# ssmit1986/BayesianInference

Measured on AMD Instinct MI355X. Metric: GP log-marg-lik evals/sec at N=32768, d=8; Cholesky TFLOP/s vs fp64 peak, higher is better.
Workload: dtype f64

## Files before the change

### bayesianinference_amd/csrc/gp_kernels.h

```cpp
#pragma once
#include <hip/hip_runtime.h>
#include <stdint.h>

#include <type_traits>

namespace gphip {

#define GP_RTC_ABI 7
#ifdef GP_D
#define GP_DIM(x) (GP_D)
#else
#define GP_DIM(x) (x)
#endif
constexpr int TB = 128;
constexpr long TS = (long)TB * TB;

__host__ __device__ __forceinline__ long tile_index(int ti, int tj, int R) {
    return (long)tj * R - ((long)tj * (tj - 1)) / 2 + (ti - tj);
}
__host__ __device__ __forceinline__ int panel_slot(int tj, int nt, int panel) {
    return tj >= nt ? (nt + panel - 1) / panel : tj / panel;
}
constexpr int SLOTP = 16;

// ... 708 lines not shown
        return sf2 * __builtin_amdgcn_exp2f(-fmaxf(u, 0.f));
    } else if (KT == 2) {
        const float q = fmaxf(u, 1e-30f);
        const float s3 = q * __builtin_amdgcn_rsqf(q);
        return sf2 * (1.0f + s3) * __builtin_amdgcn_exp2f(s3 * -1.4426950408889634f);
    } else if (KT == 3) {
        const float q = fmaxf(u, 0.f) * inv_alpha;
        return sf2 * __builtin_amdgcn_exp2f(-alpha * __builtin_amdgcn_logf(1.0f + q));
    } else {
        const float q = fmaxf(u, 1e-30f);
        const float s5 = q * __builtin_amdgcn_rsqf(q);
        return sf2 * (1.0f + s5 + q * (1.0f / 3.0f)) * __builtin_amdgcn_exp2f(s5 * -1.4426950408889634f);
    }
}

template <typename T, int KS, int KT>
__global__ __launch_bounds__(256, 2) void kbuild_mfma_kernel(KBuildMArgs<T> m) {
    const KBuildArgs<T>& a = m.b;
    constexpr int NQ = 16 / (int)sizeof(T);
    constexpr int IBR = 16 * NQ;
    constexpr int NIB = TB / IBR;
    typedef T vec_t __attribute__((ext_vector_type(NQ)));
    typedef typename Num<T>::acc_t acc_t;
    typedef typename Num<T>::pair_t pair_t;
    extern __shared__ double lds_raw[];
    const int tid = threadIdx.x, lane = tid & 63, wave = tid >> 6;
    const int slot = blockIdx.y;
    int ti, tj;
    if (a.mode == 0) {
        tri_decode(blockIdx.x + a.t0, a.nt_i, ti, tj);
    } else {
        ti = blockIdx.x % a.nt_i;
        tj = blockIdx.x / a.nt_i;
    }
    if (a.own_world > 0) {
        const int owner = (tj == a.nt_j) ? 0 : (tj / a.own_panel) % a.own_world;
        if (owner != a.own_rank) return;
    }
    const double* sp = a.slotp + (long)slot * SLOTP;
    if (sp[SP_MFMA] == 0.0) return;
    const T sf2 = (T)sp[0], sn2 = (T)sp[1], mu = (T)sp[2];
    const T alpha = (T)sp[SP_ALPHA1], inv_sf2 = (T)(1.0 / sp[0]), inv_alpha = (T)(1.0 / sp[SP_ALPHA1]);
    const T coff = (T)sp[SP_OFFSET];
    const long ldo = (a.mode == 0) ? (long)TB : a.ld;
    T* out = a.out + (long)slot * a.bstride +
             ((a.mode == 0) ? (tile_index(ti, tj, a.nt_i) + (a.adj ? a.adj[panel_slot(tj, a.nt_j, a.own_panel)] : 0l)) * TS
                            : (long)tj * TB * a.ld + (long)ti * TB);
    if (a.mode == 0 && ti == a.nt_i - 1) {
        const int r0 = 2 * lane;
        for (int jj = wave * 32; jj < wave * 32 + 32; ++jj) {
            const int gj = tj * TB + jj;
            pair_t v;
            v.x = (T)0;
            v.y = (T)0;
            if (lane == 0 && tj < a.nt_j && gj < a.n_j)
                v.x = a.y[gj] - (a.pw_mean ? a.pw_mean[(long)slot * a.pw_bstride + gj] : mu);
            *reinterpret_cast<pair_t*>(out + (long)jj * ldo + r0) = v;
        }
        return;
    }
    const int d = a.d;
    const int ks = KS > 0 ? KS : (d + 3) / 4, kr = 4 * ks;
    constexpr int KSR = KS > 0 ? KS : KB_LDS_MAXD / 4;
    constexpr bool JREG = sizeof(T) == 8;
    T* xjs = reinterpret_cast<T*>(lds_raw);
    T* xis = xjs + (JREG ? 0 : kr * KM_LDP);
    T* nrm = xis + kr * KM_LDP;
    const double* etab = reinterpret_cast<const double*>(nrm + 2 * TB);
    if (sizeof(T) == 8) {
        double* et = const_cast<double*>(etab);
        for (int idx = tid; idx < EXP_TAB; idx += 256) et[idx] = sp[0] * a.exp2tab[idx];
    }
    const double* ie = m.inv_ell + (long)slot * d;
    const double cs = KmScale<T, KT>::v;
    {
        const int side = tid >> 7, p = tid & 127;
        const T* src = side ? m.xri + (long)ti * TB + p : m.xrj + (long)tj * TB + p;
        const long np = side ? a.npad_i : a.npad_j;
        T* dst = (side ? xis : xjs) + p;
        double n2 = 0.0;
        for (int dd = 0; dd < d; ++dd) {
            const T v = (T)(((double)src[(long)dd * np] - m.centre[dd]) * (ie[dd] * cs));
            n2 = __builtin_fma((double)v, (double)v, n2);
            if (side) dst[dd * KM_LDP] = v;
            else if (!JREG) dst[dd * KM_LDP] = (T)-2 * v;
        }
        if (side || !JREG)
            for (int dd = d; dd < kr; ++dd) dst[dd * KM_LDP] = (T)0;
        nrm[side * TB + p] = (T)n2;
    }
    const int c = lane & 15, g = lane >> 4;
    T avr[2][JREG ? KSR : 1];
    if constexpr (JREG) {
#pragma unroll
        for (int jbi = 0; jbi < 2; ++jbi)
#pragma unroll
            for (int s = 0; s < KSR; ++s) {
                const int k = 4 * s + g;
                T v = (T)0;
                if (k < d)
                    v = (T)-2 * (T)(((double)m.xrj[(long)k * a.npad_j + (long)tj * TB + (wave + 4 * jbi) * 16 + c] - m.centre[k]) * (ie[k] * cs));
                avr[jbi][s] = v;
            }
    }
    __syncthreads();

    const bool edge = (a.mode == 0) ? (ti == tj || (ti + 1) * TB > a.n_i)
                                    : ((ti + 1) * TB > a.n_i || (tj + 1) * TB > a.n_j);
#pragma unroll
    for (int jbi = 0; jbi < 2; ++jbi)
#pragma unroll 1
    for (int ib = 0; ib < NIB; ++ib) {
        const int jb = wave + 4 * jbi;
        const int j0 = jb * 16, i0 = ib * IBR + NQ * c;
        const vec_t nai = *reinterpret_cast<const vec_t*>(nrm + TB + i0);
        acc_t acc[NQ];
#pragma unroll
        for (int r = 0; r < 4; ++r) {
            const T nbj = nrm[j0 + Num<T>::drow(g, r)];
#pragma unroll
            for (int q = 0; q < NQ; ++q) acc[q][r] = nai[q] + nbj;
        }
#pragma unroll
        for (int s = 0; s < KSR; ++s) {
            if (KS > 0 || s < ks) {
                const T av = JREG ? avr[jbi][JREG ? s : 0] : xjs[(4 * s + g) * KM_LDP + j0 + c];
                const vec_t bv = *reinterpret_cast<const vec_t*>(xis + (4 * s + g) * KM_LDP + i0);
#pragma unroll
                for (int q = 0; q < NQ; ++q) acc[q] = Num<T>::mfma(av, bv[q], acc[q]);
            }
        }
        const int gi0 = ti * TB + i0;
#pragma unroll
        for (int r = 0; r < 4; ++r) {
            const int jc = j0 + Num<T>::drow(g, r);
            vec_t v;
#pragma unroll
            for (int q = 0; q < NQ; ++q) v[q] = km_value<KT>(acc[q][r], sf2, etab, alpha, inv_sf2, inv_alpha) + coff;
            if (edge) {
                const int gj = tj * TB + jc;
#pragma unroll
                for (int q = 0; q < NQ; ++q) {
                    const int gi = gi0 + q;
                    if (a.mode == 0) {
                        if (gi == gj) v[q] += a.pw_nug ? a.pw_nug[(long)slot * a.pw_bstride + gj] : sn2;
                        if (gj >= a.n_j || gi >= a.n_i) v[q] = (gi == gj) ? (T)1 : (T)0;
                    } else if (gj >= a.n_j || gi >= a.n_i) {
                        v[q] = (T)0;
                    }
                }
            }
            *reinterpret_cast<vec_t*>(out + (long)jc * ldo + i0) = v;
        }
    }
}

#ifdef GPHIP_TIMING
__device__ long long* g_stamp_buf;
#define GP_STAMP(i) do { if (threadIdx.x == 0 && g_stamp_buf) g_stamp_buf[(long)blockIdx.x * 64 + (i)] = wall_clock64(); } while (0)
#else
#define GP_STAMP(i) do { } while (0)
#endif

__device__ __forceinline__ double fast_rsqrt(double x) {
    const double y = __builtin_amdgcn_rsq(x);
    const double hy = 0.5 * y;
// ... 475 lines not shown
    const long* c_adj; int c_adj_panel;
    int K;
    int r0, r1, c0, c1;
    int tri;
    int nrect;
    int ntiles;
    int swizzle;
    int super;
    int mode;
    int ktri;
    int grp_stride, grp_width, grp_count;
    int thin_row;
    int fuse_b;
    T* fuse_W; double* fuse_partial; int* fuse_info; const double* fuse_slotp; int fuse_nt;
    int skip_upper;
};

__device__ __forceinline__ void blocked_tri_decode(int p, int H, int& u, int& v) {
    const int Sf = H >> 3;
    auto prefix = [&](int J) { return (long)J * (8 * H - 28) - 32l * J * (J - 1); };
    const double b = 8.0 * H + 4.0;
    const double disc = b * b - 128.0 * (double)p;
    int J = (int)((b - __builtin_sqrt(disc > 0.0 ? disc : 0.0)) * (1.0 / 64.0));
    if (J < 0) J = 0;
    if (J > Sf) J = Sf;
    while (J > 0 && prefix(J) > p) --J;
    while (J < Sf && prefix(J + 1) <= p) ++J;
    const int q = p - (int)prefix(J);
    if (J == Sf) {
        int uu, vv;
// ... 10 lines not shown
        return;
    }
    const int below = H - 8 * J - 8, nfull = below >> 3, q2 = q - 36;
    int grp = q2 >> 6;
    if (grp < nfull) {
        const int w = q2 & 63;
        u = 8 * J + 8 + 8 * grp + (w & 7);
        v = 8 * J + (w >> 3);
    } else {
        const int rl = below & 7, w = q2 - 64 * nfull;
        u = 8 * J + 8 + 8 * nfull + w % rl;
        v = 8 * J + w / rl;
    }
}

template <typename T>
__device__ __forceinline__ void gemm_tile_decode(const GemmArgs<T>& g, int t, int r0, int c0, int nrect, int& ti, int& tj) {
    const int H = g.r1 - r0;
    if (!g.tri || t < nrect) {
        tj = c0 + t / H;
        ti = r0 + t % H;
    } else {
        int u, v;
        tri_decode(t - nrect, H, u, v);
        ti = r0 + u;
        tj = r0 + v;
    }
}

template <typename T> __device__ __forceinline__ int lds_off(int k, int row);
template <> __device__ __forceinline__ int lds_off<double>(int k, int row) { return k * LDT + row; }
template <> __device__ __forceinline__ int lds_off<float>(int k, int row) {
    return ((k >> 2) * 2 + (k & 1)) * LDP + ((k >> 1) & 1) * TB + row;
}

#ifndef GP_DIAG
#define GP_DIAG 0
#endif
template <typename T, int ROLE, int NWI, int NWJ, int NBUF>
__global__ __launch_bounds__(64 * NWI * NWJ, (NWI * NWJ == 4) ? 2 : 4) void gemm_nt_kernel(GemmArgs<T> g) {
    constexpr int NW = NWI * NWJ, FI = 8 / NWI, FJ = 8 / NWJ;
    const bool c_tiled = g.c_R > 0, a_tiled = g.a_R > 0, b_tiled = g.b_R > 0;
    extern __shared__ double smem_raw[];
    T* smem = reinterpret_cast<T*>(smem_raw);
    typedef typename Num<T>::acc_t acc_t;
    constexpr int GK = Num<T>::GK;
    constexpr int STAGE = STAGE_BYTES / (int)sizeof(T);
    constexpr int JOFF = STAGE / 2;
    constexpr bool F64 = sizeof(T) == 8;
    const int tid = threadIdx.x, lane = tid & 63, wave = tid >> 6;
    const int wi = wave % NWI, wj = wave / NWI;
    int slot = blockIdx.y;
    int bid = blockIdx.x;
    int ti, tj;
    int r0 = g.r0, c0 = g.c0, nrect = g.nrect, ntiles = g.ntiles;
// ... 16 lines not shown
        nrect = 0;
        ntiles = ntc * H - ntc * (ntc - 1) / 2;
        if (bid >= ntiles) return;
    }
    if (g.super == 2) {
        const int H = g.r1 - g.r0;
        {
            const int nx = 8, n = ntiles;
            const int q = n / nx, rem = n % nx, x = bid % nx, o = bid / nx;
            bid = (x < rem ? x * (q + 1) : rem * (q + 1) + (x - rem) * q) + o;
        }
        int u, v;
        blocked_tri_decode(bid, H, u, v);
        ti = g.r0 + u;
        tj = g.r0 + v;
    } else {
        if (g.swizzle) {
            const int nx = 8, n = ntiles;
            const int q = n / nx, rem = n % nx, x = bid % nx, o = bid / nx;
            bid = (x < rem ? x * (q + 1) : rem * (q + 1) + (x - rem) * q) + o;
        }
        gemm_tile_decode(g, bid, r0, c0, nrect, ti, tj);
    }
    ti = __builtin_amdgcn_readfirstlane(ti);
    tj = __builtin_amdgcn_readfirstlane(tj);
    slot = __builtin_amdgcn_readfirstlane(slot);

    const long koff = g.ktri ? (long)ti * TB : 0;
    const T* Abase = g.A + (long)slot * g.a_bstride;
    const T* Bbase = g.B + (long)slot * g.b_bstride;
// ... 61 lines not shown
        }
    };

    const long ldc = c_tiled ? (long)TB : g.ldc;
    T* Cg = g.C + (long)slot * g.c_bstride +
            (c_tiled ? (tile_index(ti, tj, g.c_R) + (g.c_adj ? g.c_adj[panel_slot(tj, g.c_R - 1, g.c_adj_panel)] : 0l)) * TS
                     : (long)tj * TB * g.ldc + (long)ti * TB) +
            (long)(wj * (16 * FJ)) * ldc + wi * (16 * FI) + (lane & 15);
    const int l4 = lane >> 4;
    const int nk = (g.K - (int)koff) / GK;
    const bool from_zero = (ROLE == 2) || (ROLE == 3 && g.mode == 1);
    acc_t acc[FJ][FI];
    int ny = FI;
    if (NW == 4) {
        const int uwi = uw % NWI, uwj = uw / NWI;
        if (g.thin_row == ti) ny = (uwi == 0) ? 1 : 0;
        else if (g.skip_upper && g.tri && ti == tj && uwi == 0 && uwj == 1) ny = 0;
    }
    auto load_c = [&](auto nyc) {
        constexpr int NY = decltype(nyc)::value;
#pragma unroll
        for (int x = 0; x < FJ; ++x)
#pragma unroll
            for (int y = 0; y < FI; ++y) {
                if (from_zero || (GP_DIAG & 2) || y >= NY) {
                    acc[x][y] = (acc_t){0, 0, 0, 0};
                } else {
#pragma unroll
                    for (int r = 0; r < 4; ++r)
                        acc[x][y][r] = Cg[(long)(x * 16 + Num<T>::drow(l4, r)) * ldc + y * 16];
                }
            }
    };
    auto load_frags = [&](int buf, int kk, T* fi, T* fj) {
        const T* Is = smem + buf * STAGE + wi * (16 * FI) + (lane & 15);
        const T* Js = smem + buf * STAGE + JOFF;
        const int k = 4 * kk + l4;
#pragma unroll
        for (int f = 0; f < FI; ++f) fi[f] = Is[lds_off<T>(k, f * 16)];
#pragma unroll
        for (int f = 0; f < FJ; ++f) {
            const int jrow = wj * (16 * FJ) + f * 16 + (lane & 15);
            if (ROLE == 3) {
                constexpr int G = 16 / (int)sizeof(T);
                fj[f] = Js[jrow * GK + G * ((k / G) ^ (jrow & 7)) + (k % G)];
            } else {
                fj[f] = Js[lds_off<T>(k, jrow)];
// ... 35 lines not shown
            load_frags(buf, kk, fi, fj);
            mfma_block(fi, fj, std::integral_constant<int, FI>{}, kb * GK + 4 * kk);
        }
    };
    if constexpr (NBUF == 2) {
        constexpr int NKK = GK / 4;
        static_assert(NKK % 2 == 0, "fragment set parity must repeat every stage");
        auto pipeline = [&](auto nyc) {
            constexpr int NY = decltype(nyc)::value;
            T fa[2][FI], fb[2][FJ];
#ifdef GP_STAGGER
            if (ROLE == 0 && (blockIdx.x & 256) && blockIdx.x < 512)
                for (int i = 0; i < GP_STAGGER; ++i) __builtin_amdgcn_s_sleep(127);
#endif
            stage(0, 0);
            load_c(nyc);
            asm volatile("s_waitcnt vmcnt(0)" ::: "memory");
            __syncthreads();
            if (NY > 0) load_frags(0, 0, fa[0], fb[0]);
            for (int kb = 0; kb < nk; ++kb) {
                const int cur = kb & 1;
                if (kb + 1 < nk && !((GP_DIAG & 1) && kb >= 1)) stage(kb + 1, cur ^ 1);
                if (NY > 0) {
#pragma unroll
                    for (int kk = 0; kk + 1 < NKK; ++kk) {
                        pin_frags(fa[kk & 1], fb[kk & 1]);
                        __builtin_amdgcn_sched_barrier(0);
                        load_frags(cur, kk + 1, fa[(kk + 1) & 1], fb[(kk + 1) & 1]);
                        __builtin_amdgcn_sched_barrier(0);
                        mfma_block(fa[kk & 1], fb[kk & 1], nyc, kb * GK + 4 * kk);
                        __builtin_amdgcn_sched_barrier(0);
// ... 1310 lines not shown
```

### bayesianinference_amd/csrc/gphip.hip

```cpp
#include "gp_kernels.h"
#include "gp_trsv.h"
#include "rccl_dyn.h"
#include "rtc_dyn.h"

#include <hip/hip_ext.h>

#include <algorithm>
#include <chrono>
#include <cctype>
#include <cmath>
#include <cstdio>
#include <cstdlib>
#include <cstring>
#include <mutex>
#include <string>
#include <vector>

#include "../../include/gphip.h"

using namespace gphip;

namespace {

constexpr double LOG_TWO_PI = 1.8378770664093454835606594728112;
// ... 93 lines not shown
    Buf dExp2;
    Buf dCentre;
    std::vector<double> x_centre, x_half;
    int kbuild_mfma = 1, kbuild_mfma_bound = 512, kbuild_mfma_digits = 9;
    double test_ratio = 0.0;
    int slots = 0;
    Buf dA, dXs, dW;
    Buf dDinv;
    Buf dW64;
    unsigned long w64_gen = ~0ul;
    Buf dLT, dW64T;
    unsigned long lt_gen = ~0ul;
    Buf dInvEll, dSlotp, dPartial, dRes, dInfo;
    Buf hInvEll, hSlotp, hRes, hInfo;
    int panel = 4, profile = 0, swizzle = 1, max_slots = 256, lookahead = 1;
    int supertile = 2;
    int latency_gemm = 1;
    static constexpr int latency_tiles = 256;
    int latency_max_nt = 48;
    int dataflow = 1, dataflow_max_nt = 96;
    int dataflow_max_slots = -1;
    int dataflow_max_tasks = 34000;
    int dataflow_fine_nt = 96;
    int panel_left = -1;
    int fuse_option = 1;
    int grad_potri = 1;
    int grad_batch_slots = 0;
    int grad_batch_max_n = 7168;
    int grad_batch_last = 0, grad_batch_route = 0;
    Buf dKinvB;
    int predict_df_max_nt = 256;
// ... 362 lines not shown
bool use_dataflow(const gphip_ctx* h, int nslots);
inline int few_slots(const gphip_ctx* h) { return h->dataflow_max_slots < 0 ? 8 : h->dataflow_max_slots; }
hipEvent_t sync_event(gphip_ctx* h);

void queue_custom_prep(gphip_ctx* h, int nslots) {
    if (!h->custom) return;
    const void* x = h->dXt.p;
    int npad = (int)h->Npad, n = (int)h->N, d = (int)h->d, ncp = std::max(h->ncp, 1);
    const double* cp = h->dCustomP.as<double>();
    double* sp = h->dSlotp.as<double>();
    void* params[] = {&x, &npad, &n, &d, &cp, &ncp, &sp};
    (void)hipModuleLaunchKernel(h->f_cprep, (unsigned)nslots, 1, 1, 256, 1, 1, 0, h->cs, params, nullptr);
}

template <typename T>
int queue_build(gphip_ctx* h, int nslots) {
    const long tot = (long)h->d * h->Npad;
    int gx = (int)((tot + 255) / 256);
    if (gx > 1024) gx = 1024;
    if (h->theta_packed) {
        ThetaPack tp;
        memcpy(tp.v, h->hInvEll.as<double>(), (size_t)nslots * h->d * 8);
        memcpy(tp.v + (size_t)nslots * h->d, h->hSlotp.as<double>(), (size_t)nslots * SLOTP * 8);
        hipLaunchKernelGGL(k_scale_theta<T>, dim3(gx, nslots), dim3(256), 0, h->cs, (const T*)h->dXt.p, (T*)h->dXs.p, tp,
                           h->dInvEll.as<double>(), h->dSlotp.as<double>(), h->dInfo.as<int>(), (int)h->d, (int)h->Npad, nslots);
    } else {
        hipLaunchKernelGGL(k_scale<T>, dim3(gx, nslots), dim3(256), 0, h->cs, (const T*)h->dXt.p, (T*)h->dXs.p,
                           h->dInvEll.as<double>(), (int)h->d, (int)h->Npad);
    }
    if (h->nl2 > 0)
        hipLaunchKernelGGL(k_scale<T>, dim3(gx, nslots), dim3(256), 0, h->cs, (const T*)h->dXt.p, (T*)h->dXs2.p, h->dInvEll2.as<double>(),
                           (int)h->d, (int)h->Npad);
    queue_custom_prep(h, nslots);
    KBuildArgs<T> a{};
    a.ks = h->ks; a.xi2 = a.xj2 = (const T*)h->dXs2.p;
    a.out = (T*)h->dA.p; a.ld = TB; a.bstride = h->slot_elems;
    a.xi = (const T*)h->dXs.p; a.xj = (const T*)h->dXs.p; a.xi_bstride = a.xj_bstride = tot;
    a.npad_i = a.npad_j = (int)h->Npad; a.n_i = a.n_j = (int)h->N;
    a.y = (const T*)h->dY.p; a.slotp = h->dSlotp.as<double>(); a.d = (int)h->d; a.mode = 0; a.exp2tab = h->dExp2.as<double>();
    a.nt_i = (int)h->Nt + 1; a.nt_j = (int)h->Nt;
    a.own_panel = h->panel; a.own_world = h->dist_world; a.own_rank = h->dist_rank;
    if (h->dist_world > 0) { a.out = (T*)h->dist_base; a.adj = h->dDistAdj.as<long>(); }
    a.pw_nug = h->pw_nug_on ? (const T*)h->dPwNug.p : nullptr;
    a.pw_mean = h->pw_mean_on ? (const T*)h->dPwMean.p : nullptr;
    a.pw_bstride = h->Npad;
    const long ntiles = (long)(h->Nt + 1) * (h->Nt + 2) / 2;
    ProfScope ps(h, 0, 0.0, (double)sizeof(T) * nslots * ((double)h->N * (h->N + 1) / 2 + (double)h->N * h->d));
    launch_kbuild<T>(h, a, dim3((unsigned)ntiles, nslots), (const T*)h->dXt.p, (const T*)h->dXt.p);
    return 0;
}

template <typename T>
struct Opnd {
    const T* p; long ld; long bs; int R; int k0;
    const long* adj = nullptr; int adj_panel = 0;
    int lower = 0;
};
template <typename T>
Opnd<T> cm(const T* p, long ld, long bs) { return Opnd<T>{p, ld, bs, 0, 0}; }
template <typename T>
Opnd<T> wb(const T* W, int b, long lrs) {
    Opnd<T> o{W + (long)b * TB * TB - (long)b * TB, TB, lrs, 0, 0};
    o.lower = 1;
    return o;
}
template <typename T>
Opnd<T> tl(const gphip_ctx* h, int k0 = 0, bool all_slots = true) {
    return Opnd<T>{(const T*)(h->ws_override ? h->ws_override : h->dA.p), TB, all_slots ? (long)h->slot_elems : 0l, (int)h->R, k0};
}

template <typename T>
size_t potrf_lds();

template <typename T>
bool launch_gemm(gphip_ctx* h, int cls, Opnd<T> Co, Opnd<T> Ao, Opnd<T> Bo, int K, int r0, int r1, int c0, int c1, int tri,
                 int nslots, int mode = 0, int ktri = 0, int thin_row = -1, int fuse_b = -1, int groups = 1, int grp_stride = 0,
                 int grp_width = 0) {
    GemmArgs<T> g{};
    g.grp_stride = groups > 1 ? grp_stride : 0;
    g.grp_width = grp_width;
    g.grp_count = groups;
    g.mode = mode;
    g.ktri = ktri;
    g.thin_row = h->thin_tiles ? thin_row : -1;
    g.skip_upper = (h->thin_tiles && thin_row >= 0 && tri && mode == 0 && !ktri) ? 1 : 0;
    g.C = const_cast<T*>(Co.p); g.ldc = Co.ld; g.c_bstride = Co.bs; g.c_R = Co.R;
    g.c_adj = Co.adj; g.c_adj_panel = Co.adj_panel;
    g.b_lower = Bo.lower;
    g.A = Ao.p; g.lda = Ao.ld; g.a_bstride = Ao.bs; g.a_R = Ao.R; g.a_k0 = Ao.k0;
    g.B = Bo.p; g.ldb = Bo.ld; g.b_bstride = Bo.bs; g.b_R = Bo.R; g.b_k0 = Bo.k0;
    g.K = K; g.r0 = r0; g.r1 = r1; g.c0 = c0; g.c1 = c1; g.tri = tri;
    const int H = r1 - r0, W = c1 - c0;
    if (H <= 0 || W <= 0) return false;
    if (!tri) {
        g.nrect = H * W;
        g.ntiles = H * W;
    } else {
        int nrc = r0 - c0;
        if (nrc > W) nrc = W;
        const int ntc = W - nrc;
        g.nrect = nrc * H;
        g.ntiles = g.nrect + ntc * H - ntc * (ntc - 1) / 2;
    }
    g.swizzle = h->swizzle && g.ntiles >= 64 && !ktri;
    int grid_x = g.ntiles;
    if (tri && r0 == c0 && W == H && h->supertile >= 2 && H >= 16 && mode == 0 && groups == 1 && (nslots == 1 || h->supertile == 3)) {
        g.super = 2;
    }
    double flops = 2.0 * TB * TB * (double)K * g.ntiles * nslots;
    if (g.grp_stride > 0) {
        double fl = 0.0;
        long tiles = 0;
        for (int q = 0; q < groups; ++q) {
            const int a0 = c0 + q * grp_stride, a1 = std::min(a0 + grp_width, c1);
            const int Hq = r1 - a0, wq = a1 - a0;
            tiles += (long)wq * Hq - (long)wq * (wq - 1) / 2;
            const double a = (double)a0 * TB, b = std::min((double)a1 * TB, (double)h->N);
            const double cnt = b > a ? b - a : 0.0;
            fl += 2.0 * (double)K * (cnt * (double)h->N - (a + b - 1.0) * cnt / 2.0);
        }
        long dense = 0;
        for (int q = 0; q < groups; ++q) {
            const int a0 = c0 + q * grp_stride, wq = std::min(grp_width, c1 - a0), Hq = r1 - a0;
            dense += (long)wq * Hq - (long)wq * (wq - 1) / 2;
        }
        g.nrect = 0;
        g.ntiles = (int)dense;
        flops = cls == 4 ? fl : 2.0 * TB * TB * (double)K * (double)tiles;
    } else if (cls == 4 && tri && r0 == c0) {
        const double a = (double)c0 * TB, b = std::min((double)c1 * TB, (double)h->N);
        const double cnt = b > a ? b - a : 0.0;
        flops = 2.0 * (double)K * (cnt * (double)h->N - (a + b - 1.0) * cnt / 2.0) * nslots;
    }
    const double bytes = (double)sizeof(T) * nslots * (2.0 * TB * TB * g.ntiles + (double)(tri ? H : H + W) * TB * K);
    ProfScope ps(h, cls == 6 ? 3 : cls, flops, bytes);
    const dim3 grid(g.grp_stride > 0 ? (unsigned)g.ntiles : (unsigned)grid_x, g.grp_stride > 0 ? 1u : (unsigned)nslots);
    const bool lat = h->latency_gemm && !g.super && h->Nt <= h->latency_max_nt && (long)grid_x * nslots <= h->latency_tiles;
    g.fuse_b = -1;
    size_t lds2 = GEMM_LDS;
    if (fuse_b >= 0 && cls == 3 && mode == 0 && !lat && !ktri && groups == 1 && tri && fuse_b >= c0 && fuse_b < c1 && fuse_b >= r0) {
        g.fuse_b = fuse_b;
        g.fuse_W = (T*)h->dW.p; g.fuse_partial = h->dPartial.as<double>(); g.fuse_info = h->dInfo.as<int>(); g.fuse_slotp = h->dSlotp.as<double>(); g.fuse_nt = (int)h->Nt;
        lds2 = std::max(lds2, potrf_lds<T>());
    }
#define GEMM_LAUNCH(ROLE)                                                                                          \
    do {                                                                                                           \
        if (lat) hipLaunchKernelGGL((gemm_nt_kernel<T, ROLE, 4, 4, 4>), grid, dim3(1024), 2 * GEMM_LDS, h->cs, g);  \
        else hipLaunchKernelGGL((gemm_nt_kernel<T, ROLE, 2, 2, 2>), grid, dim3(256), GEMM_LDS, h->cs, g);           \
    } while (0)
    if (cls == 6) GEMM_LAUNCH(3);
    else if (mode == 1) GEMM_LAUNCH(2);
    else if (cls == 4) GEMM_LAUNCH(0);
    else if (g.fuse_b >= 0) hipLaunchKernelGGL((gemm_nt_kernel<T, 4, 2, 2, 2>), grid, dim3(256), lds2, h->cs, g);
    else GEMM_LAUNCH(1);
#undef GEMM_LAUNCH
    return g.fuse_b >= 0;
}

hipEvent_t sync_event(gphip_ctx* h) {
    if (h->sync_used == h->sync_events.size()) {
        hipEvent_t e = nullptr;
        if (hipEventCreateWithFlags(&e, hipEventDisableTiming) != hipSuccess) return nullptr;
        h->sync_events.push_back(e);
    }
    return h->sync_events[h->sync_used++];
// ... 267 lines not shown
    if (h->Nt <= 48) launch_dataflow<T, 128, 1, 4>(h, nslots);
    else launch_dataflow<T, 128, 1>(h, nslots);
    launch_finalize<T>(h, nslots, (int)h->Nt);
    if (h->want_u && nslots == 1) launch_dataflow_inverse<T, 128, 1>(h);
    return 0;
}

template <typename T>
int queue_factor(gphip_ctx* h, int nslots) {
    const int Nt = (int)h->Nt, R = Nt + 1;
    const std::vector<int> bnd = panel_bounds(h);
    const int nouter = (int)bnd.size() - 1;
    auto k0 = [&](int k) { return bnd[(size_t)std::min(k, nouter)]; };
    auto trailing = [&](int k, int c_lo, int c_hi, int cls, int fuse_b = -1) {
        return launch_gemm<T>(h, cls, tl<T>(h), tl<T>(h, k0(k)), tl<T>(h, k0(k)), (k0(k + 1) - k0(k)) * TB, c_lo, R, c_lo, c_hi, 1,
                              nslots, 0, 0, Nt, fuse_b);
    };
    if (use_dataflow(h, nslots)) return queue_factor_dataflow<T>(h, nslots);
    double* tail_part = nullptr;
    int tail_n = 0, tail_k0 = -1;
    bool pdf = false;
    if constexpr (sizeof(T) == 8) pdf = panel_df_on(h, nslots) && nouter >= 2;
    auto df_panel = [&](int kp, int kprev) {
        if constexpr (sizeof(T) == 8) {
            const int c0 = 2 * (kprev >= 0 ? k0(kprev) : k0(kp));
            launch_dataflow<T, 64>(h, 1, c0, nullptr, 0, 2 * k0(kp + 1) - c0, kprev >= 0 ? 2 * (k0(kp) - k0(kprev)) : 0, h->dA.p);
        }
    };
    if (!h->lookahead || nouter < 2) {
        for (int k = 0; k < nouter; ++k) {
            queue_panel<T>(h, k0(k), k0(k + 1) - k0(k), nslots);
// ... 304 lines not shown
        okv[s] = stage_theta(h, s, Theta + (size_t)s * h->p, h->pw_nug_host ? h->pw_nug_host + (size_t)(s0 + s) * h->N : nullptr,
                             h->pw_mean_host ? h->pw_mean_host + (size_t)(s0 + s) * h->N : nullptr);
    {
        const int rc = upload_pw(h, s0, nb);
        if (rc) return rc;
    }
    h->theta_packed = h->kt != 2 && (size_t)nb * (h->d + SLOTP) <= (size_t)THETA_PACK;
    if (!h->theta_packed) {
        const int rc = copy_theta(h, nb);
        if (rc) return rc;
        HIPCHK(hipMemsetAsync(h->dInfo.p, 0, (size_t)nb * 4, h->stream));
    }
    h->fused_eval = h->fuse_option && h->theta_packed && h->kt != 2 && h->dtype == 64 && !h->want_w && h->profile < 2 &&
                    !h->pw_mean_on && !h->pw_nug_on && use_dataflow(h, nb) && h->Nt <= h->dataflow_fine_nt;
    {
        ProfScope ps(h, 5, 0.0, 0.0);
        if (!h->fused_eval) DISPATCH(h, queue_build, h, nb);
        DISPATCH(h, queue_factor, h, nb);
    }
    h->fused_eval = false;
    h->theta_packed = false;
    h->pw_mean_on = h->pw_nug_on = false;
    HIPCHK(hipStreamSynchronize(h->stream));
    HIPCHK(hipGetLastError());
    harvest(h);
    if (h->hInfo.as<int>()[nb] != 0 && getenv("GPHIP_DEBUG")) {
        fprintf(stderr, "gphip debug: nb=%d hInfo[nb]=%d slots=%d; hInfo[0..]:", nb, h->hInfo.as<int>()[nb], h->slots);
        for (int i = 0; i <= nb && i < 80; ++i) fprintf(stderr, " %d", h->hInfo.as<int>()[i]);
        fprintf(stderr, "\n");
    }
// ... 64 lines not shown
                                   hipFuncAttributeMaxDynamicSharedMemorySize,
                                   (int)((4 * h->d + 1) * TB * sizeof(T) + 8 + 4 * (2 * h->d + 6) * 8)));
        HIPCHK(hipFuncSetAttribute(reinterpret_cast<const void*>(grad_reduce_general_slots_kernel<T>),
                                   hipFuncAttributeMaxDynamicSharedMemorySize,
                                   (int)((4 * h->d + 1) * TB * sizeof(T) + 8 + 4 * (2 * h->d + 6) * 8)));
    }
#define GEMM_ATTR(ROLE)                                                                                   \
    HIPCHK(hipFuncSetAttribute(reinterpret_cast<const void*>(gemm_nt_kernel<T, ROLE, 2, 2, 2>),             \
                               hipFuncAttributeMaxDynamicSharedMemorySize, (int)GEMM_LDS));                  \
    HIPCHK(hipFuncSetAttribute(reinterpret_cast<const void*>(gemm_nt_kernel<T, ROLE, 4, 4, 4>),             \
                               hipFuncAttributeMaxDynamicSharedMemorySize, (int)(2 * GEMM_LDS)));
    GEMM_ATTR(0) GEMM_ATTR(1) GEMM_ATTR(2) GEMM_ATTR(3)
#undef GEMM_ATTR
    HIPCHK(hipFuncSetAttribute(reinterpret_cast<const void*>(gemm_nt_kernel<T, 4, 2, 2, 2>),
                               hipFuncAttributeMaxDynamicSharedMemorySize, (int)std::max(GEMM_LDS, potrf_lds<T>())));
    return GPHIP_OK;
}

template <typename T>
int upload(gphip_ctx* h, void* dst, const std::vector<double>& src, hipStream_t st) {
    if (sizeof(T) == 8) {
        HIPCHK(hipMemcpyAsync(dst, src.data(), src.size() * 8, hipMemcpyHostToDevice, st));
        HIPCHK(hipStreamSynchronize(st));
    } else {
        std::vector<float> tmp(src.begin(), src.end());
        HIPCHK(hipMemcpyAsync(dst, tmp.data(), tmp.size() * 4, hipMemcpyHostToDevice, st));
        HIPCHK(hipStreamSynchronize(st));
    }
    return GPHIP_OK;
}
// ... 1843 lines not shown
        return fail(h, GPHIP_ERR_HIP, "dataflow panel schedule timed out (set option dist_panel_df=0 and report)");
    }
    *logdet_partial = h->hRes.as<double>()[0];
    *quad = (h->dist_rank == 0) ? h->hRes.as<double>()[1] : 0.0;
    *info = h->dist_theta_ok ? h->hInfo.as<int>()[0] : GPHIP_INFO_NAN;
    h->dist_world = 0; h->dist_rank = 0;
    return GPHIP_OK;
}

namespace {
int* option_slot(gphip_ctx* h, const char* name) {
    struct Entry { const char* name; int gphip_ctx::*field; };
    static const Entry table[] = {
        {"panel", &gphip_ctx::panel}, {"profile", &gphip_ctx::profile}, {"xcd_swizzle", &gphip_ctx::swizzle},
        {"lookahead", &gphip_ctx::lookahead}, {"supertile", &gphip_ctx::supertile}, {"panel_wide", &gphip_ctx::panel_wide},
        {"panel_left", &gphip_ctx::panel_left}, {"thin_tiles", &gphip_ctx::thin_tiles}, {"fuse_potrf", &gphip_ctx::fuse_potrf},
        {"latency_gemm", &gphip_ctx::latency_gemm}, {"latency_max_nt", &gphip_ctx::latency_max_nt},
        {"dataflow", &gphip_ctx::dataflow}, {"dataflow_max_nt", &gphip_ctx::dataflow_max_nt},
        {"dataflow_max_slots", &gphip_ctx::dataflow_max_slots}, {"dataflow_max_tasks", &gphip_ctx::dataflow_max_tasks}, {"dataflow_fine_nt", &gphip_ctx::dataflow_fine_nt},
        {"dataflow_tail", &gphip_ctx::dataflow_tail}, {"dataflow_lds_kib", &gphip_ctx::dataflow_lds_kib},
        {"dataflow_occ3", &gphip_ctx::dataflow_occ3},
        {"fused_eval", &gphip_ctx::fuse_option}, {"panel_df", &gphip_ctx::panel_df}, {"grad_potri", &gphip_ctx::grad_potri}, {"predict_df", &gphip_ctx::predict_df},
        {"kbuild_mfma", &gphip_ctx::kbuild_mfma}, {"kbuild_mfma_bound", &gphip_ctx::kbuild_mfma_bound},
        {"kbuild_mfma_digits", &gphip_ctx::kbuild_mfma_digits}, {"trsv", &gphip_ctx::trsv}, {"predict_df_max_nt", &gphip_ctx::predict_df_max_nt}, {"last_issue_us", &gphip_ctx::last_issue_us}, {"last_dist_panel_df", &gphip_ctx::dist_df_mode},
        {"custom_grad", &gphip_ctx::custom_grad}, {"grad_analytic", &gphip_ctx::grad_analytic},
        {"grad_batch_slots", &gphip_ctx::grad_batch_slots}, {"last_grad_batch_slots", &gphip_ctx::grad_batch_last},
        {"last_grad_batch_route", &gphip_ctx::grad_batch_route}, {"grad_batch_max_n", &gphip_ctx::grad_batch_max_n},
        {"max_slots", &gphip_ctx::max_slots}, {"shard_min_n", &gphip_ctx::shard_min_n},
        {"replicate_factor", &gphip_ctx::replicate_factor}, {"share_local_panels", &gphip_ctx::share_local_panels},
        {"bcast_chunks", &gphip_ctx::bcast_chunks}, {"bcast_two_hop", &gphip_ctx::bcast_two_hop}, {"dist_panel_df", &gphip_ctx::dist_panel_df}, {"dist_owner_yield", &gphip_ctx::dist_owner_yield},
// ... 112 lines not shown
```

Before: 5.565.

## Add aligned supertile trailing-GEMM order and optional first-touch fused kernel build

```diff
diff --git a/bayesianinference_amd/csrc/gp_kernels.h b/bayesianinference_amd/csrc/gp_kernels.h
--- a/bayesianinference_amd/csrc/gp_kernels.h
+++ b/bayesianinference_amd/csrc/gp_kernels.h
@@ -746,6 +746,91 @@
     }
 }
 
+template <typename T> struct KmSlot { T sf2, sn2, mu, alpha, inv_sf2, inv_alpha, coff; };
+template <typename T>
+__device__ __forceinline__ KmSlot<T> km_slot(const double* sp) {
+    KmSlot<T> s;
+    s.sf2 = (T)sp[0]; s.sn2 = (T)sp[1]; s.mu = (T)sp[2];
+    s.alpha = (T)sp[SP_ALPHA1]; s.inv_sf2 = (T)(1.0 / sp[0]); s.inv_alpha = (T)(1.0 / sp[SP_ALPHA1]);
+    s.coff = (T)sp[SP_OFFSET];
+    return s;
+}
+template <typename T, bool JLDS>
+__device__ __forceinline__ void km_stage(const KBuildMArgs<T>& m, int slot, int ti, int tj, int kr, double cs, int tid,
+                                         T* xjs, T* xis, T* nrm, double* et) {
+    const KBuildArgs<T>& a = m.b;
+    const double* sp = a.slotp + (long)slot * SLOTP;
+    const int d = a.d;
+    if (sizeof(T) == 8) {
+        for (int idx = tid; idx < EXP_TAB; idx += 256) et[idx] = sp[0] * a.exp2tab[idx];
+    }
+    const double* ie = m.inv_ell + (long)slot * d;
+    const int side = tid >> 7, p = tid & 127;
+    const T* src = side ? m.xri + (long)ti * TB + p : m.xrj + (long)tj * TB + p;
+    const long np = side ? a.npad_i : a.npad_j;
+    T* dst = (side ? xis : xjs) + p;
+    double n2 = 0.0;
+    for (int dd = 0; dd < d; ++dd) {
+        const T v = (T)(((double)src[(long)dd * np] - m.centre[dd]) * (ie[dd] * cs));
+        n2 = __builtin_fma((double)v, (double)v, n2);
+        if (side) dst[dd * KM_LDP] = v;
+        else if (JLDS) dst[dd * KM_LDP] = (T)-2 * v;
+    }
+    if (side || JLDS)
+        for (int dd = d; dd < kr; ++dd) dst[dd * KM_LDP] = (T)0;
+    nrm[side * TB + p] = (T)n2;
+}
+template <typename T, int NQ>
+__device__ __forceinline__ void km_load(const T* p, T (&o)[NQ]) {
+    if constexpr (NQ == 1) {
+        o[0] = p[0];
+    } else {
+        typedef T vec_t __attribute__((ext_vector_type(NQ)));
+        const vec_t v = *reinterpret_cast<const vec_t*>(p);
+#pragma unroll
+        for (int q = 0; q < NQ; ++q) o[q] = v[q];
+    }
+}
+template <typename T, int NQ, int KSR, bool KSTATIC, class AV>
+__device__ __forceinline__ void km_block_u(typename Num<T>::acc_t (&acc)[NQ], const T* nrm, const T* xis, int i0, int j0, int g, int ks, AV av) {
+    T nai[NQ];
+    km_load<T, NQ>(nrm + TB + i0, nai);
+#pragma unroll
+    for (int r = 0; r < 4; ++r) {
+        const T nbj = nrm[j0 + Num<T>::drow(g, r)];
+#pragma unroll
+        for (int q = 0; q < NQ; ++q) acc[q][r] = nai[q] + nbj;
+    }
+#pragma unroll
+    for (int s = 0; s < KSR; ++s) {
+        if (KSTATIC || s < ks) {
+            const T avs = av(s);
+            T bv[NQ];
+            km_load<T, NQ>(xis + (4 * s + g) * KM_LDP + i0, bv);
+#pragma unroll
+            for (int q = 0; q < NQ; ++q) acc[q] = Num<T>::mfma(avs, bv[q], acc[q]);
+        }
+    }
+}
+template <typename T, int KT>
+__device__ __forceinline__ T km_entry(T u, const KmSlot<T>& s, const double* etab, const KBuildArgs<T>& a, int slot, bool edge, int gi, int gj) {
+    T v = km_value<KT>(u, s.sf2, etab, s.alpha, s.inv_sf2, s.inv_alpha) + s.coff;
+    if (edge) {
+        if (a.mode == 0) {
+            if (gi == gj) v += a.pw_nug ? a.pw_nug[(long)slot * a.pw_bstride + gj] : s.sn2;
+            if (gj >= a.n_j || gi >= a.n_i) v = (gi == gj) ? (T)1 : (T)0;
+        } else if (gj >= a.n_j || gi >= a.n_i) {
+            v = (T)0;
+        }
+    }
+    return v;
+}
+template <typename T>
+__device__ __forceinline__ T km_rhs(const KBuildArgs<T>& a, int slot, int tj, int gj, T mu) {
+    if (tj < a.nt_j && gj < a.n_j) return a.y[gj] - (a.pw_mean ? a.pw_mean[(long)slot * a.pw_bstride + gj] : mu);
+    return (T)0;
+}
+
 template <typename T, int KS, int KT>
 __global__ __launch_bounds__(256, 2) void kbuild_mfma_kernel(KBuildMArgs<T> m) {
     const KBuildArgs<T>& a = m.b;
@@ -771,9 +856,7 @@
     }
     const double* sp = a.slotp + (long)slot * SLOTP;
     if (sp[SP_MFMA] == 0.0) return;
-    const T sf2 = (T)sp[0], sn2 = (T)sp[1], mu = (T)sp[2];
-    const T alpha = (T)sp[SP_ALPHA1], inv_sf2 = (T)(1.0 / sp[0]), inv_alpha = (T)(1.0 / sp[SP_ALPHA1]);
-    const T coff = (T)sp[SP_OFFSET];
+    const KmSlot<T> ksl = km_slot<T>(sp);
     const long ldo = (a.mode == 0) ? (long)TB : a.ld;
     T* out = a.out + (long)slot * a.bstride +
              ((a.mode == 0) ? (tile_index(ti, tj, a.nt_i) + (a.adj ? a.adj[panel_slot(tj, a.nt_j, a.own_panel)] : 0l)) * TS
@@ -781,12 +864,10 @@
     if (a.mode == 0 && ti == a.nt_i - 1) {
         const int r0 = 2 * lane;
         for (int jj = wave * 32; jj < wave * 32 + 32; ++jj) {
-            const int gj = tj * TB + jj;
             pair_t v;
             v.x = (T)0;
             v.y = (T)0;
-            if (lane == 0 && tj < a.nt_j && gj < a.n_j)
-                v.x = a.y[gj] - (a.pw_mean ? a.pw_mean[(long)slot * a.pw_bstride + gj] : mu);
+            if (lane == 0) v.x = km_rhs<T>(a, slot, tj, tj * TB + jj, ksl.mu);
             *reinterpret_cast<pair_t*>(out + (long)jj * ldo + r0) = v;
         }
         return;
@@ -799,28 +880,9 @@
     T* xis = xjs + (JREG ? 0 : kr * KM_LDP);
     T* nrm = xis + kr * KM_LDP;
     const double* etab = reinterpret_cast<const double*>(nrm + 2 * TB);
-    if (sizeof(T) == 8) {
-        double* et = const_cast<double*>(etab);
-        for (int idx = tid; idx < EXP_TAB; idx += 256) et[idx] = sp[0] * a.exp2tab[idx];
-    }
     const double* ie = m.inv_ell + (long)slot * d;
     const double cs = KmScale<T, KT>::v;
-    {
-        const int side = tid >> 7, p = tid & 127;
-        const T* src = side ? m.xri + (long)ti * TB + p : m.xrj + (long)tj * TB + p;
-        const long np = side ? a.npad_i : a.npad_j;
-        T* dst = (side ? xis : xjs) + p;
-        double n2 = 0.0;
-        for (int dd = 0; dd < d; ++dd) {
-            const T v = (T)(((double)src[(long)dd * np] - m.centre[dd]) * (ie[dd] * cs));
-            n2 = __builtin_fma((double)v, (double)v, n2);
-            if (side) dst[dd * KM_LDP] = v;
-            else if (!JREG) dst[dd * KM_LDP] = (T)-2 * v;
-        }
-        if (side || !JREG)
-            for (int dd = d; dd < kr; ++dd) dst[dd * KM_LDP] = (T)0;
-        nrm[side * TB + p] = (T)n2;
-    }
+    km_stage<T, !JREG>(m, slot, ti, tj, kr, cs, tid, xjs, xis, nrm, const_cast<double*>(etab));
     const int c = lane & 15, g = lane >> 4;
     T avr[2][JREG ? KSR : 1];
     if constexpr (JREG) {
@@ -845,43 +907,16 @@
     for (int ib = 0; ib < NIB; ++ib) {
         const int jb = wave + 4 * jbi;
         const int j0 = jb * 16, i0 = ib * IBR + NQ * c;
-        const vec_t nai = *reinterpret_cast<const vec_t*>(nrm + TB + i0);
         acc_t acc[NQ];
-#pragma unroll
-        for (int r = 0; r < 4; ++r) {
-            const T nbj = nrm[j0 + Num<T>::drow(g, r)];
-#pragma unroll
-            for (int q = 0; q < NQ; ++q) acc[q][r] = nai[q] + nbj;
-        }
-#pragma unroll
-        for (int s = 0; s < KSR; ++s) {
-            if (KS > 0 || s < ks) {
-                const T av = JREG ? avr[jbi][JREG ? s : 0] : xjs[(4 * s + g) * KM_LDP + j0 + c];
-                const vec_t bv = *reinterpret_cast<const vec_t*>(xis + (4 * s + g) * KM_LDP + i0);
-#pragma unroll
-                for (int q = 0; q < NQ; ++q) acc[q] = Num<T>::mfma(av, bv[q], acc[q]);
-            }
-        }
+        km_block_u<T, NQ, KSR, (KS > 0)>(acc, nrm, xis, i0, j0, g, ks,
+                                         [&](int s) { return JREG ? avr[jbi][JREG ? s : 0] : xjs[(4 * s + g) * KM_LDP + j0 + c]; });
         const int gi0 = ti * TB + i0;
 #pragma unroll
         for (int r = 0; r < 4; ++r) {
             const int jc = j0 + Num<T>::drow(g, r);
             vec_t v;
 #pragma unroll
-            for (int q = 0; q < NQ; ++q) v[q] = km_value<KT>(acc[q][r], sf2, etab, alpha, inv_sf2, inv_alpha) + coff;
-            if (edge) {
-                const int gj = tj * TB + jc;
-#pragma unroll
-                for (int q = 0; q < NQ; ++q) {
-                    const int gi = gi0 + q;
-                    if (a.mode == 0) {
-                        if (gi == gj) v[q] += a.pw_nug ? a.pw_nug[(long)slot * a.pw_bstride + gj] : sn2;
-                        if (gj >= a.n_j || gi >= a.n_i) v[q] = (gi == gj) ? (T)1 : (T)0;
-                    } else if (gj >= a.n_j || gi >= a.n_i) {
-                        v[q] = (T)0;
-                    }
-                }
-            }
+            for (int q = 0; q < NQ; ++q) v[q] = km_entry<T, KT>(acc[q][r], ksl, etab, a, slot, edge, gi0 + q, tj * TB + jc);
             *reinterpret_cast<vec_t*>(out + (long)jc * ldo + i0) = v;
         }
     }
@@ -1387,6 +1422,7 @@
     int fuse_b;
     T* fuse_W; double* fuse_partial; int* fuse_info; const double* fuse_slotp; int fuse_nt;
     int skip_upper;
+    KBuildMArgs<T> ft; int ft_kt;
 };
 
 __device__ __forceinline__ void blocked_tri_decode(int p, int H, int& u, int& v) {
@@ -1427,6 +1463,52 @@
     }
 }
 
+__device__ __forceinline__ void aligned_tri_decode(int bid, int H, int& u, int& v) {
+    const int Hm = H - 1, Sf = Hm >> 3, rl = Hm & 7, x = bid & 7;
+    const int F = Sf * (Sf - 1) / 2, Fd = F & ~7;
+    auto full_super = [&](int f, int w) {
+        int I, J;
+        tri_decode(f, Sf - 1, I, J);
+        u = 8 * (I + 1) + (w & 7);
+        v = 8 * J + (w >> 3);
+    };
+    int lo = 64 * Fd;
+    if (bid < lo) {
+        const int o = bid >> 3;
+        full_super((o >> 6) * 8 + x, o & 63);
+        return;
+    }
+    auto below = [&](int m) { return (m >> 3) * x + ((m & 7) < x ? (m & 7) : x); };
+    auto index = [&](int hi) { return below(hi) - below(lo) + ((bid - lo) >> 3); };
+    const int nA = 64 * (F - Fd), nB = 8 * rl * Sf, nC = 28 * Sf + rl * (rl - 1) / 2;
+    if (bid < lo + nA + nB + nC) {
+        int p = index(lo + nA + nB + nC);
+        if (p < nA) {
+            full_super(Fd + (p >> 6), p & 63);
+        } else if (p < nA + nB) {
+            p -= nA;
+            const int J = p / (8 * rl), w = p % (8 * rl);
+            u = 8 * Sf + w % rl;
+            v = 8 * J + w / rl;
+        } else {
+            p -= nA + nB;
+            const int J = p / 28 < Sf ? p / 28 : Sf;
+            tri_decode(p - 28 * J, J < Sf ? 7 : rl - 1, u, v);
+            u += 8 * J + 1;
+            v += 8 * J;
+        }
+        return;
+    }
+    lo += nA + nB + nC;
+    if (bid < lo + Hm) {
+        u = v = index(lo + Hm);
+        return;
+    }
+    lo += Hm;
+    u = H - 1;
+    v = index(lo + H);
+}
+
 template <typename T>
 __device__ __forceinline__ void gemm_tile_decode(const GemmArgs<T>& g, int t, int r0, int c0, int nrect, int& ti, int& tj) {
     const int H = g.r1 - r0;
@@ -1450,8 +1532,13 @@
 #ifndef GP_DIAG
 #define GP_DIAG 0
 #endif
-template <typename T, int ROLE, int NWI, int NWJ, int NBUF>
+constexpr int FT_MAX_D = 12;
+static_assert((2 * FT_MAX_D * KM_LDP + 2 * TB) * 8 + EXP_TAB * 8 <= STAGE_BYTES, "first-touch point image must fit one stage");
+template <typename T, int ROLE_, int NWI, int NWJ, int NBUF>
 __global__ __launch_bounds__(64 * NWI * NWJ, (NWI * NWJ == 4) ? 2 : 4) void gemm_nt_kernel(GemmArgs<T> g) {
+    constexpr bool FT = ROLE_ >= 5;
+    constexpr int ROLE = ROLE_ == 5 ? 0 : (ROLE_ == 6 ? 4 : ROLE_);
+    static_assert(!FT || (sizeof(T) == 8 && NWI == 2 && NWJ == 2 && NBUF == 2), "first-touch roles: fp64, 2x2 waves, two stages");
     constexpr int NW = NWI * NWJ, FI = 8 / NWI, FJ = 8 / NWJ;
     const bool c_tiled = g.c_R > 0, a_tiled = g.a_R > 0, b_tiled = g.b_R > 0;
     extern __shared__ double smem_raw[];
@@ -1498,6 +1585,11 @@
         blocked_tri_decode(bid, H, u, v);
         ti = g.r0 + u;
         tj = g.r0 + v;
+    } else if (g.super == 4) {
+        int u, v;
+        aligned_tri_decode(bid, g.r1 - g.r0, u, v);
+        ti = g.r0 + u;
+        tj = g.r0 + v;
     } else {
         if (g.swizzle) {
             const int nx = 8, n = ntiles;
@@ -1589,7 +1681,7 @@
     int ny = FI;
     if (NW == 4) {
         const int uwi = uw % NWI, uwj = uw / NWI;
-        if (g.thin_row == ti) ny = (uwi == 0) ? 1 : 0;
+        if (g.thin_row == ti) ny = FT ? FI : ((uwi == 0) ? 1 : 0);
         else if (g.skip_upper && g.tri && ti == tj && uwi == 0 && uwj == 1) ny = 0;
     }
     auto load_c = [&](auto nyc) {
@@ -1606,6 +1698,65 @@
                         acc[x][y][r] = Cg[(long)(x * 16 + Num<T>::drow(l4, r)) * ldc + y * 16];
                 }
             }
+    };
+    auto build_c = [&](auto nyc) {
+        constexpr int NY = decltype(nyc)::value;
+        if constexpr (FT) {
+            const KBuildArgs<T>& a = g.ft.b;
+            const int d = a.d, ks = (d + 3) / 4, kr = 4 * ks;
+            T* xjs = smem + STAGE;
+            T* xis = xjs + kr * KM_LDP;
+            T* nrm = xis + kr * KM_LDP;
+            double* etab = reinterpret_cast<double*>(nrm + 2 * TB);
+            const KmSlot<T> ksl = km_slot<T>(a.slotp + (long)slot * SLOTP);
+            const bool rhs = ti == a.nt_i - 1;
+            if (!rhs) {
+                const int kt = g.ft_kt;
+                const double cs = kt == 0 ? KmScale<T, 0>::v : (kt == 1 ? KmScale<T, 1>::v : (kt == 2 ? KmScale<T, 2>::v : KmScale<T, 3>::v));
+                km_stage<T, true>(g.ft, slot, ti, tj, kr, cs, tid, xjs, xis, nrm, etab);
+            }
+            __syncthreads();
+            const int c = lane & 15;
+            const bool edge = ti == tj || (ti + 1) * TB > a.n_i;
+            auto entries = [&](auto ktc) {
+                constexpr int KT = decltype(ktc)::value;
+#pragma unroll
+                for (int x = 0; x < FJ; ++x)
+#pragma unroll
+                    for (int y = 0; y < FI; ++y) {
+                        if (y >= NY) {
+                            acc[x][y] = (acc_t){0, 0, 0, 0};
+                            continue;
+                        }
+                        const int i0 = wi * (16 * FI) + y * 16 + c, j0 = wj * (16 * FJ) + x * 16;
+                        acc_t u[1];
+                        km_block_u<T, 1, (FT_MAX_D + 3) / 4, false>(u, nrm, xis, i0, j0, l4, ks,
+                                                                    [&](int s) { return xjs[(4 * s + l4) * KM_LDP + j0 + c]; });
+#pragma unroll
+                        for (int r = 0; r < 4; ++r)
+                            acc[x][y][r] = km_entry<T, KT>(u[0][r], ksl, etab, a, slot, edge, ti * TB + i0, tj * TB + j0 + Num<T>::drow(l4, r));
+#pragma unroll
+                        for (int r = 0; r < 4; ++r) asm volatile("" : "+v"(acc[x][y][r]));
+                        __builtin_amdgcn_sched_barrier(0);
+                    }
+            };
+            if (rhs) {
+#pragma unroll
+                for (int x = 0; x < FJ; ++x)
+#pragma unroll
+                    for (int y = 0; y < FI; ++y) {
+                        acc[x][y] = (acc_t){0, 0, 0, 0};
+                        if (y < NY && wi * (16 * FI) + y * 16 + c == 0) {
+#pragma unroll
+                            for (int r = 0; r < 4; ++r)
+                                acc[x][y][r] = km_rhs<T>(a, slot, tj, tj * TB + wj * (16 * FJ) + x * 16 + Num<T>::drow(l4, r), ksl.mu);
+                        }
+                    }
+            } else if (g.ft_kt == 0) entries(std::integral_constant<int, 0>{});
+            else if (g.ft_kt == 1) entries(std::integral_constant<int, 1>{});
+            else if (g.ft_kt == 2) entries(std::integral_constant<int, 2>{});
+            else entries(std::integral_constant<int, 3>{});
+        }
     };
     auto load_frags = [&](int buf, int kk, T* fi, T* fj) {
         const T* Is = smem + buf * STAGE + wi * (16 * FI) + (lane & 15);
@@ -1671,7 +1822,8 @@
                 for (int i = 0; i < GP_STAGGER; ++i) __builtin_amdgcn_s_sleep(127);
 #endif
             stage(0, 0);
-            load_c(nyc);
+            if constexpr (FT) build_c(nyc);
+            else load_c(nyc);
             asm volatile("s_waitcnt vmcnt(0)" ::: "memory");
             __syncthreads();
             if (NY > 0) load_frags(0, 0, fa[0], fb[0]);
diff --git a/bayesianinference_amd/csrc/gphip.hip b/bayesianinference_amd/csrc/gphip.hip
--- a/bayesianinference_amd/csrc/gphip.hip
+++ b/bayesianinference_amd/csrc/gphip.hip
@@ -131,7 +131,10 @@
     Buf dInvEll, dSlotp, dPartial, dRes, dInfo;
     Buf hInvEll, hSlotp, hRes, hInfo;
     int panel = 4, profile = 0, swizzle = 1, max_slots = 256, lookahead = 1;
-    int supertile = 2;
+    int supertile = 4;
+    int first_touch_build = 0;
+    bool ft_on = false;
+    int ft_last = 0;
     int latency_gemm = 1;
     static constexpr int latency_tiles = 256;
     int latency_max_nt = 48;
@@ -524,6 +527,34 @@
 }
 
 template <typename T>
+KBuildArgs<T> workspace_build_args(const gphip_ctx* h) {
+    const long tot = (long)h->d * h->Npad;
+    KBuildArgs<T> a{};
+    a.ks = h->ks; a.xi2 = a.xj2 = (const T*)h->dXs2.p;
+    a.out = (T*)h->dA.p; a.ld = TB; a.bstride = h->slot_elems;
+    a.xi = (const T*)h->dXs.p; a.xj = (const T*)h->dXs.p; a.xi_bstride = a.xj_bstride = tot;
+    a.npad_i = a.npad_j = (int)h->Npad; a.n_i = a.n_j = (int)h->N;
+    a.y = (const T*)h->dY.p; a.slotp = h->dSlotp.as<double>(); a.d = (int)h->d; a.mode = 0; a.exp2tab = h->dExp2.as<double>();
+    a.nt_i = (int)h->Nt + 1; a.nt_j = (int)h->Nt;
+    a.own_panel = h->panel; a.own_world = h->dist_world; a.own_rank = h->dist_rank;
+    if (h->dist_world > 0) { a.out = (T*)h->dist_base; a.adj = h->dDistAdj.as<long>(); }
+    a.pw_nug = h->pw_nug_on ? (const T*)h->dPwNug.p : nullptr;
+    a.pw_mean = h->pw_mean_on ? (const T*)h->dPwMean.p : nullptr;
+    a.pw_bstride = h->Npad;
+    return a;
+}
+
+bool panel_df_on(const gphip_ctx* h, int nslots);
+bool first_touch_applies(const gphip_ctx* h, int nb) {
+    if (!h->first_touch_build || h->dtype != 64 || h->custom || h->dist_world > 0 || h->ws_override || h->fused_eval) return false;
+    if (nb > few_slots(h) || use_dataflow(h, nb) || panel_df_on(h, nb)) return false;
+    if (h->pw_mean_on || h->pw_nug_on || mfma_family(h) < 0 || h->d > FT_MAX_D || !h->dCentre.p) return false;
+    for (int s2 = 0; s2 < nb; ++s2)
+        if (h->hSlotp.as<double>()[(size_t)s2 * SLOTP + SP_MFMA] == 0.0) return false;
+    return true;
+}
+
+template <typename T>
 int queue_build(gphip_ctx* h, int nslots) {
     const long tot = (long)h->d * h->Npad;
     int gx = (int)((tot + 255) / 256);
@@ -542,20 +573,16 @@
         hipLaunchKernelGGL(k_scale<T>, dim3(gx, nslots), dim3(256), 0, h->cs, (const T*)h->dXt.p, (T*)h->dXs2.p, h->dInvEll2.as<double>(),
                            (int)h->d, (int)h->Npad);
     queue_custom_prep(h, nslots);
-    KBuildArgs<T> a{};
-    a.ks = h->ks; a.xi2 = a.xj2 = (const T*)h->dXs2.p;
-    a.out = (T*)h->dA.p; a.ld = TB; a.bstride = h->slot_elems;
-    a.xi = (const T*)h->dXs.p; a.xj = (const T*)h->dXs.p; a.xi_bstride = a.xj_bstride = tot;
-    a.npad_i = a.npad_j = (int)h->Npad; a.n_i = a.n_j = (int)h->N;
-    a.y = (const T*)h->dY.p; a.slotp = h->dSlotp.as<double>(); a.d = (int)h->d; a.mode = 0; a.exp2tab = h->dExp2.as<double>();
-    a.nt_i = (int)h->Nt + 1; a.nt_j = (int)h->Nt;
-    a.own_panel = h->panel; a.own_world = h->dist_world; a.own_rank = h->dist_rank;
-    if (h->dist_world > 0) { a.out = (T*)h->dist_base; a.adj = h->dDistAdj.as<long>(); }
-    a.pw_nug = h->pw_nug_on ? (const T*)h->dPwNug.p : nullptr;
-    a.pw_mean = h->pw_mean_on ? (const T*)h->dPwMean.p : nullptr;
-    a.pw_bstride = h->Npad;
-    const long ntiles = (long)(h->Nt + 1) * (h->Nt + 2) / 2;
-    ProfScope ps(h, 0, 0.0, (double)sizeof(T) * nslots * ((double)h->N * (h->N + 1) / 2 + (double)h->N * h->d));
+    const KBuildArgs<T> a = workspace_build_args<T>(h);
+    long ntiles = (long)(h->Nt + 1) * (h->Nt + 2) / 2;
+    double entries = (double)h->N * (h->N + 1) / 2;
+    if (h->ft_on) {
+        const long w = panel_bounds(h)[1], R = h->Nt + 1;
+        ntiles = w * R - w * (w - 1) / 2;
+        const double c = std::min((double)w * TB, (double)h->N);
+        entries = c * (double)h->N - c * (c - 1.0) / 2.0;
+    }
+    ProfScope ps(h, 0, 0.0, (double)sizeof(T) * nslots * (entries + (double)h->N * h->d));
     launch_kbuild<T>(h, a, dim3((unsigned)ntiles, nslots), (const T*)h->dXt.p, (const T*)h->dXt.p);
     return 0;
 }
@@ -585,7 +612,7 @@
 template <typename T>
 bool launch_gemm(gphip_ctx* h, int cls, Opnd<T> Co, Opnd<T> Ao, Opnd<T> Bo, int K, int r0, int r1, int c0, int c1, int tri,
                  int nslots, int mode = 0, int ktri = 0, int thin_row = -1, int fuse_b = -1, int groups = 1, int grp_stride = 0,
-                 int grp_width = 0) {
+                 int grp_width = 0, bool first_touch = false) {
     GemmArgs<T> g{};
     g.grp_stride = groups > 1 ? grp_stride : 0;
     g.grp_width = grp_width;
@@ -616,6 +643,7 @@
     int grid_x = g.ntiles;
     if (tri && r0 == c0 && W == H && h->supertile >= 2 && H >= 16 && mode == 0 && groups == 1 && (nslots == 1 || h->supertile == 3)) {
         g.super = 2;
+        if (h->supertile == 4 && thin_row == r1 - 1 && !ktri) g.super = 4;
     }
     double flops = 2.0 * TB * TB * (double)K * g.ntiles * nslots;
     if (g.grp_stride > 0) {
@@ -645,7 +673,7 @@
     const double bytes = (double)sizeof(T) * nslots * (2.0 * TB * TB * g.ntiles + (double)(tri ? H : H + W) * TB * K);
     ProfScope ps(h, cls == 6 ? 3 : cls, flops, bytes);
     const dim3 grid(g.grp_stride > 0 ? (unsigned)g.ntiles : (unsigned)grid_x, g.grp_stride > 0 ? 1u : (unsigned)nslots);
-    const bool lat = h->latency_gemm && !g.super && h->Nt <= h->latency_max_nt && (long)grid_x * nslots <= h->latency_tiles;
+    const bool lat = h->latency_gemm && !g.super && h->Nt <= h->latency_max_nt && (long)grid_x * nslots <= h->latency_tiles && !first_touch;
     g.fuse_b = -1;
     size_t lds2 = GEMM_LDS;
     if (fuse_b >= 0 && cls == 3 && mode == 0 && !lat && !ktri && groups == 1 && tri && fuse_b >= c0 && fuse_b < c1 && fuse_b >= r0) {
@@ -658,7 +686,16 @@
         if (lat) hipLaunchKernelGGL((gemm_nt_kernel<T, ROLE, 4, 4, 4>), grid, dim3(1024), 2 * GEMM_LDS, h->cs, g);  \
         else hipLaunchKernelGGL((gemm_nt_kernel<T, ROLE, 2, 2, 2>), grid, dim3(256), GEMM_LDS, h->cs, g);           \
     } while (0)
-    if (cls == 6) GEMM_LAUNCH(3);
+    if (first_touch) {
+        if constexpr (sizeof(T) == 8) {
+            g.ft.b = workspace_build_args<T>(h);
+            g.ft.xri = g.ft.xrj = (const T*)h->dXt.p;
+            g.ft.inv_ell = h->dInvEll.as<double>(); g.ft.centre = h->dCentre.as<double>();
+            g.ft_kt = mfma_family(h);
+            if (cls == 4) hipLaunchKernelGGL((gemm_nt_kernel<T, 5, 2, 2, 2>), grid, dim3(256), GEMM_LDS, h->cs, g);
+            else hipLaunchKernelGGL((gemm_nt_kernel<T, 6, 2, 2, 2>), grid, dim3(256), lds2, h->cs, g);
+        }
+    } else if (cls == 6) GEMM_LAUNCH(3);
     else if (mode == 1) GEMM_LAUNCH(2);
     else if (cls == 4) GEMM_LAUNCH(0);
     else if (g.fuse_b >= 0) hipLaunchKernelGGL((gemm_nt_kernel<T, 4, 2, 2, 2>), grid, dim3(256), lds2, h->cs, g);
@@ -956,7 +993,7 @@
     auto k0 = [&](int k) { return bnd[(size_t)std::min(k, nouter)]; };
     auto trailing = [&](int k, int c_lo, int c_hi, int cls, int fuse_b = -1) {
         return launch_gemm<T>(h, cls, tl<T>(h), tl<T>(h, k0(k)), tl<T>(h, k0(k)), (k0(k + 1) - k0(k)) * TB, c_lo, R, c_lo, c_hi, 1,
-                              nslots, 0, 0, Nt, fuse_b);
+                              nslots, 0, 0, Nt, fuse_b, 1, 0, 0, h->ft_on && k == 0);
     };
     if (use_dataflow(h, nslots)) return queue_factor_dataflow<T>(h, nslots);
     double* tail_part = nullptr;
@@ -1291,6 +1328,8 @@
     h->fused_eval = h->fuse_option && h->theta_packed && h->kt != 2 && h->dtype == 64 && !h->want_w && h->profile < 2 &&
                     !h->pw_mean_on && !h->pw_nug_on && use_dataflow(h, nb) && h->Nt <= h->dataflow_fine_nt;
     {
+        Scoped<bool> ft(h->ft_on, first_touch_applies(h, nb));
+        h->ft_last = h->ft_on ? 1 : 0;
         ProfScope ps(h, 5, 0.0, 0.0);
         if (!h->fused_eval) DISPATCH(h, queue_build, h, nb);
         DISPATCH(h, queue_factor, h, nb);
@@ -1385,6 +1424,12 @@
 #undef GEMM_ATTR
     HIPCHK(hipFuncSetAttribute(reinterpret_cast<const void*>(gemm_nt_kernel<T, 4, 2, 2, 2>),
                                hipFuncAttributeMaxDynamicSharedMemorySize, (int)std::max(GEMM_LDS, potrf_lds<T>())));
+    if constexpr (sizeof(T) == 8) {
+        HIPCHK(hipFuncSetAttribute(reinterpret_cast<const void*>(gemm_nt_kernel<T, 5, 2, 2, 2>),
+                                   hipFuncAttributeMaxDynamicSharedMemorySize, (int)GEMM_LDS));
+        HIPCHK(hipFuncSetAttribute(reinterpret_cast<const void*>(gemm_nt_kernel<T, 6, 2, 2, 2>),
+                                   hipFuncAttributeMaxDynamicSharedMemorySize, (int)std::max(GEMM_LDS, potrf_lds<T>())));
+    }
     return GPHIP_OK;
 }
 
@@ -3258,6 +3303,7 @@
     static const Entry table[] = {
         {"panel", &gphip_ctx::panel}, {"profile", &gphip_ctx::profile}, {"xcd_swizzle", &gphip_ctx::swizzle},
         {"lookahead", &gphip_ctx::lookahead}, {"supertile", &gphip_ctx::supertile}, {"panel_wide", &gphip_ctx::panel_wide},
+        {"first_touch_build", &gphip_ctx::first_touch_build}, {"last_first_touch", &gphip_ctx::ft_last},
         {"panel_left", &gphip_ctx::panel_left}, {"thin_tiles", &gphip_ctx::thin_tiles}, {"fuse_potrf", &gphip_ctx::fuse_potrf},
         {"latency_gemm", &gphip_ctx::latency_gemm}, {"latency_max_nt", &gphip_ctx::latency_max_nt},
         {"dataflow", &gphip_ctx::dataflow}, {"dataflow_max_nt", &gphip_ctx::dataflow_max_nt},
```

New measurement: 5.584 (median of 6 runs). Within noise of the previous version (+0.3%).
